# RenYurui/Global-Flow-Local-Attention

Hardware: AMD Instinct MI355X
Metric: images/sec (fwd+bwd) PoseGenerator 256x176 attn_layer=2,3 -- feature-warping hot path (higher is better)
Workload: dtype f32 (FC products: 2-term f16 splits exact to 2^-24 on f16 MFMA, f32 accumulate)

## Files before the change

### global_flow_local_attention_amd/csrc/patch_mfma.hip

```cpp
#include "gfla_common.h"
#include "patch_mfma.h"
#include "rs_taps.h"

namespace gfla {

typedef float pm_f32x16 __attribute__((ext_vector_type(16)));

struct PatchEntry {
  int q;
  float v;
};

constexpr int kPmStatSlots = 32;
constexpr int kPmTile = 32;
constexpr int kPmSub = 8;
constexpr int kPmChannels = 128;
constexpr int kPmMaxNB = 6;
constexpr int kPmGPitch = 33;

struct PmLayout {
  int64_t ntiles, table_bytes, rows_bytes, total;
};
static PmLayout pm_layout(int64_t B, int64_t HW, int entries) {
  PmLayout L;
  L.ntiles = ceil_div(HW, kPmTile);
  L.table_bytes = ((B * L.ntiles * kPmTile * entries * (int64_t)sizeof(PatchEntry)) + 255) & ~(int64_t)255;
  L.rows_bytes = ((B * L.ntiles * (int64_t)sizeof(int2)) + 255) & ~(int64_t)255;
  L.total = L.table_bytes + L.rows_bytes + 256;
  return L;
}

__device__ __forceinline__ unsigned pm_stat_total(const unsigned *stat) {
  unsigned tot = 0;
#pragma unroll
  for (int i = 0; i < kPmStatSlots; ++i) tot += stat[i];
  return tot;
}

__device__ __forceinline__ int pm_safe_int(float v) {
  return (int)fminf(fmaxf(v, -1048576.f), 1048576.f);
}

__device__ __forceinline__ void pm_store_tile_rows(int lo, int hi, int2 *slot, unsigned *stat) {
  __shared__ int s_lo[4], s_hi[4];
#pragma unroll
  for (int m = 32; m >= 1; m >>= 1) {
    lo = min(lo, __shfl_xor(lo, m));
    hi = max(hi, __shfl_xor(hi, m));
  }
  if ((threadIdx.x & 63) == 0) {
    s_lo[threadIdx.x >> 6] = lo;
    s_hi[threadIdx.x >> 6] = hi;
  }
  __syncthreads();
  if (threadIdx.x == 0) {
    const int l = min(min(s_lo[0], s_lo[1]), min(s_lo[2], s_lo[3])), h = max(max(s_hi[0], s_hi[1]), max(s_hi[2], s_hi[3]));
    *slot = make_int2(l, h);
    if (h >= l) atomicAdd(stat + (blockIdx.x + blockIdx.y * gridDim.x) % kPmStatSlots, (unsigned)(h - l + 1));
  }
}

struct Fold {
  int r_lo, r_hi, s_lo, s_hi, ty, tx;
  bool canonical;
};
__device__ __forceinline__ Fold pm_fold(int r, int s, int y0, int x0, int P, int Hs, int Ws) {
  Fold f;
  const int yy = y0 + r, xx = x0 + s;
  f.r_lo = f.r_hi = r;
  f.s_lo = f.s_hi = s;
  f.canonical = true;
  if (yy <= 0) {
    f.r_lo = 0;
    f.canonical = f.canonical && (yy == 0 || r == P - 1);
  } else if (yy >= Hs - 1) {
    f.r_hi = P - 1;
    f.canonical = f.canonical && (yy == Hs - 1 || r == 0);
  }
  if (xx <= 0) {
    f.s_lo = 0;
    f.canonical = f.canonical && (xx == 0 || s == P - 1);
  } else if (xx >= Ws - 1) {
    f.s_hi = P - 1;
    f.canonical = f.canonical && (xx == Ws - 1 || s == 0);
  }
  f.ty = clampi(yy, 0, Hs - 1);
  f.tx = clampi(xx, 0, Ws - 1);
  return f;
}

template <int K>
struct AggTaps {
  float fx0, fy0;
  int xf, yf, x0, y0;
  bool dense;
  __device__ __forceinline__ float dx(int t) const { return (fx0 + (float)(t - K / 2)) + (float)xf; }
  __device__ __forceinline__ float dy(int t) const { return (fy0 + (float)(t - K / 2)) + (float)yf; }
  __device__ __forceinline__ float ax(int t) const { const float d = dx(t); return d - floorf(d); }
  __device__ __forceinline__ float ay(int t) const { const float d = dy(t); return d - floorf(d); }
  __device__ __forceinline__ void init(float fx, float fy, int x, int y) {
    fx0 = fx, fy0 = fy, xf = x, yf = y;
    dense = true;
    x0 = y0 = 0;
#pragma unroll
    for (int t = 0; t < K; ++t) {
      const int ix = (int)floorf(dx(t)), iy = (int)floorf(dy(t));
      if (t == 0) x0 = ix, y0 = iy;
      dense = dense && (ix == x0 + t) && (iy == y0 + t);
    }
  }
};

template <int K>
__global__ __launch_bounds__(256) void agg_patch_table_kernel(const float *__restrict__ flow,
                                                             const float *__restrict__ attn,
                                                             PatchEntry *__restrict__ table,
                                                             int2 *__restrict__ tile_rows,
                                                             unsigned *__restrict__ stat, int H, int W, int Hs, int Ws,
                                                             int ntiles) {
  constexpr int P = K + 1, E = P * P, KK = K * K;
  static_assert(E % 2 == 0, "entries are written two at a time");
  typedef int i32x4 __attribute__((ext_vector_type(4)));
  const int64_t b = blockIdx.y;
  const int HW = H * W;
  const int tile = blockIdx.x * 8 + (threadIdx.x >> 5), pl = threadIdx.x & 31;
  if (tile >= ntiles) return;
  const int p = tile * kPmTile + pl;
  const float inv_kk = 1.f / (float)KK;
  int lo = 0x7fffffff, hi = -1;
  i32x4 *out = reinterpret_cast<i32x4 *>(table + ((b * ntiles + tile) * kPmTile + pl) * (int64_t)E);
  bool dense = false;
  AggTaps<K> tp;
  if (p < HW) {
    const int yf = p / W, xf = p - yf * W;
    tp.init(flow[(b * 2 + 0) * HW + p], flow[(b * 2 + 1) * HW + p], xf, yf);
    dense = tp.dense;
  }
  if (dense) {
    const int y0 = pm_safe_int((float)tp.y0), x0 = pm_safe_int((float)tp.x0);
    lo = clampi(y0, 0, Hs - 1);
    hi = clampi(y0 + K, 0, Hs - 1);
    float a[KK];
    const float *at = attn + b * (int64_t)KK * HW + p;
#pragma unroll
    for (int t = 0; t < KK; ++t) a[t] = at[(int64_t)t * HW] * inv_kk;
    float ax[K], ay[K];
#pragma unroll
    for (int t = 0; t < K; ++t) {
      ax[t] = tp.ax(t);
      ay[t] = tp.ay(t);
    }
    float v[P][P];
#pragma unroll
    for (int r = 0; r < P; ++r) {
#pragma unroll
      for (int q = 0; q < P; ++q) v[r][q] = 0.f;
#pragma unroll
      for (int j = 0; j < K; ++j) {
        float wrow = 0.f;
        if (r < K) wrow += a[r * K + j] * (1.f - ay[r]);
        if (r > 0) wrow += a[(r - 1) * K + j] * ay[r - 1];
        v[r][j] += wrow * (1.f - ax[j]);
        v[r][j + 1] += wrow * ax[j];
      }
    }
    int clo[P], chi[P], rlo[P], rhi[P], tx[P], ty[P];
    bool ccan[P], rcan[P];
#pragma unroll
    for (int i = 0; i < P; ++i) {
      const int xx = x0 + i, yy = y0 + i;
      clo[i] = chi[i] = rlo[i] = rhi[i] = i;
      ccan[i] = rcan[i] = true;
      if (xx <= 0) {
        clo[i] = 0;
        ccan[i] = xx == 0 || i == P - 1;
      } else if (xx >= Ws - 1) {
        chi[i] = P - 1;
        ccan[i] = xx == Ws - 1 || i == 0;
      }
      if (yy <= 0) {
        rlo[i] = 0;
        rcan[i] = yy == 0 || i == P - 1;
      } else if (yy >= Hs - 1) {
        rhi[i] = P - 1;
        rcan[i] = yy == Hs - 1 || i == 0;
      }
      tx[i] = clampi(xx, 0, Ws - 1);
      ty[i] = clampi(yy, 0, Hs - 1);
    }
    float cf[P][P];
#pragma unroll
    for (int r = 0; r < P; ++r)
#pragma unroll
      for (int q = 0; q < P; ++q) {
        float acc = 0.f;
#pragma unroll
        for (int q2 = 0; q2 < P; ++q2) acc += (q2 >= clo[q] && q2 <= chi[q]) ? v[r][q2] : 0.f;
        cf[r][q] = acc;
      }
#pragma unroll
    for (int r = 0; r < P; ++r)
#pragma unroll
      for (int q = 0; q < P; q += 2) {
        float acc0 = 0.f, acc1 = 0.f;
#pragma unroll
        for (int r2 = 0; r2 < P; ++r2) {
          const bool in = r2 >= rlo[r] && r2 <= rhi[r];
          acc0 += in ? cf[r2][q] : 0.f;
          acc1 += in ? cf[r2][q + 1] : 0.f;
        }
        const bool c0 = rcan[r] && ccan[q], c1 = rcan[r] && ccan[q + 1];
        i32x4 e;
        e.x = c0 ? (ty[r] << 16) | tx[q] : -1;
        e.y = c0 ? __float_as_int(acc0) : 0;
        e.z = c1 ? (ty[r] << 16) | tx[q + 1] : -1;
        e.w = c1 ? __float_as_int(acc1) : 0;
        out[(r * P + q) >> 1] = e;
      }
  } else {
    const i32x4 none = {-1, 0, -1, 0};
#pragma unroll
    for (int e = 0; e < E / 2; ++e) out[e] = none;
  }
#pragma unroll
  for (int msk = 16; msk >= 1; msk >>= 1) {
    lo = min(lo, __shfl_xor(lo, msk));
    hi = max(hi, __shfl_xor(hi, msk));
  }
  if (pl == 0) {
    tile_rows[b * ntiles + tile] = make_int2(lo, hi);
    if (hi >= lo) atomicAdd(stat + (tile + (int)b * ntiles) % kPmStatSlots, (unsigned)(hi - lo + 1));
  }
}

template <int K>
__global__ __launch_bounds__(256) void agg_scatter_nondense_kernel(const float *__restrict__ flow,
                                                                  const float *__restrict__ attn,
                                                                  const float *__restrict__ gout,
                                                                  float *__restrict__ gsrc, int C, int H, int W,
                                                                  int Hs, int Ws, const unsigned *__restrict__ stat,
                                                                  unsigned limit) {
  constexpr int KK = K * K;
  const int HW = H * W;
  if (pm_stat_total(stat) > limit) return;
  const int p = blockIdx.x * 256 + threadIdx.x;
  const int64_t b = blockIdx.y;
  if (p >= HW) return;
  const int yf = p / W, xf = p - yf * W;
  AggTaps<K> tp;
  tp.init(flow[(b * 2 + 0) * HW + p], flow[(b * 2 + 1) * HW + p], xf, yf);
  if (tp.dense) return;
  const float *at = attn + b * (int64_t)KK * HW + p;
  const float inv_kk = 1.f / (float)KK;
  for (int c = 0; c < C; ++c) {
    const float go = gout[(b * C + c) * (int64_t)HW + p] * inv_kk;
    float *gp = gsrc + (b * C + c) * (int64_t)Hs * Ws;
#pragma unroll 1
    for (int i = 0; i < K; ++i) {
      const float dy = tp.dy(i), fdy = floorf(dy);
      const int yT = clampi(pm_safe_int(fdy), 0, Hs - 1) * Ws, yB = clampi(pm_safe_int(fdy + 1), 0, Hs - 1) * Ws;
      const float yB_P = dy - fdy, yT_P = 1.f - yB_P;
#pragma unroll 1
      for (int j = 0; j < K; ++j) {
        const float dx = tp.dx(j), fdx = floorf(dx);
        const int xL = clampi(pm_safe_int(fdx), 0, Ws - 1), xR = clampi(pm_safe_int(fdx + 1), 0, Ws - 1);
        const float xR_P = dx - fdx, xL_P = 1.f - xR_P;
        const float gv = at[(int64_t)(i * K + j) * HW] * go;
        atomic_add(gp + yT + xL, gv * xL_P * yT_P);
        atomic_add(gp + yT + xR, gv * xR_P * yT_P);
        atomic_add(gp + yB + xL, gv * xL_P * yB_P);
        atomic_add(gp + yB + xR, gv * xR_P * yB_P);
      }
    }
  }
}

template <int KH>
__global__ __launch_bounds__(256) void rs_patch_table_kernel(const float *__restrict__ in2,
                                                            PatchEntry *__restrict__ table,
                                                            int2 *__restrict__ tile_rows,
                                                            unsigned *__restrict__ stat, int H, int W, int Hi, int Wi,
                                                            int trunc) {
  constexpr int P = 2 * KH, E = P * P;
  const int tile = blockIdx.x, ntiles = gridDim.x;
  const int64_t b = blockIdx.y;
  const int HW = H * W;
  const int pl = threadIdx.x >> 3, sub = threadIdx.x & (kPmSub - 1);
  const int p = tile * kPmTile + pl;
  PatchEntry *out = table + ((b * ntiles + tile) * kPmTile + pl) * (int64_t)E;
  int lo = 0x7fffffff, hi = -1;
  if (p < HW) {
    const int y = p / W, x = p - y * W;
    const float *i2 = in2 + b * 3 * (int64_t)HW + p;
    Taps<float, KH> t;
    t.template init<2>(i2[0], i2[HW], i2[2 * (int64_t)HW], x, y, Hi, Wi, 1, trunc != 0);
    const int y0 = pm_safe_int((float)t.iy0) - (KH - 1), x0 = pm_safe_int((float)t.ix0) - (KH - 1);
    lo = clampi(y0, 0, Hi - 1);
    hi = clampi(y0 + P - 1, 0, Hi - 1);
    float wy[P], wx[P];
#pragma unroll
    for (int r = 0; r < P; ++r) {
      wy[r] = (float)safe_div<float>(t.row_w(r), t.sum);
      wx[r] = t.col_w(r);
    }
    for (int e = sub; e < E; e += kPmSub) {
      const int r = e / P, s = e - r * P;
      const Fold f = pm_fold(r, s, y0, x0, P, Hi, Wi);
      float v = 0.f;
      if (f.canonical) {
#pragma unroll
        for (int rr = 0; rr < P; ++rr)
#pragma unroll
          for (int ss = 0; ss < P; ++ss)
            if (rr >= f.r_lo && rr <= f.r_hi && ss >= f.s_lo && ss <= f.s_hi) v += wy[rr] * wx[ss];
      }
      out[e] = f.canonical ? PatchEntry{(f.ty << 16) | f.tx, v} : PatchEntry{-1, 0.f};
    }
  } else {
    for (int e = sub; e < E; e += kPmSub) out[e] = PatchEntry{-1, 0.f};
  }
  pm_store_tile_rows(lo, hi, tile_rows + b * ntiles + tile, stat);
}

constexpr int kPmMaxEntriesPerThread = 5;

typedef float pm_f32x4 __attribute__((ext_vector_type(4)));

__device__ __forceinline__ void pm_fetch(pm_f32x4 (&gv)[4], int (&peq)[kPmMaxEntriesPerThread],
                                         float (&pev)[kPmMaxEntriesPerThread], int tile, const float *g_row, bool g_ok,
                                         bool g_vec, int gh, int HW, const PatchEntry *tab, int sub, int E) {
  const int pbase = tile * kPmTile + gh * 16;
#pragma unroll
  for (int q = 0; q < 4; ++q) {
    const int p = pbase + 4 * q;
    pm_f32x4 v = {0.f, 0.f, 0.f, 0.f};
    if (g_ok) {
      const float *src = g_row + (int64_t)tile * kPmTile + 4 * q;
      if (g_vec && p + 3 < HW) {
        v = *reinterpret_cast<const pm_f32x4 *>(src);
      } else {
        if (p < HW) v[0] = src[0];
        if (p + 1 < HW) v[1] = src[1];
        if (p + 2 < HW) v[2] = src[2];
        if (p + 3 < HW) v[3] = src[3];
      }
    }
    gv[q] = v;
  }
  const unsigned long long *tp = reinterpret_cast<const unsigned long long *>(tab + (int64_t)tile * kPmTile * E);
#pragma unroll
  for (int m = 0; m < kPmMaxEntriesPerThread; ++m) {
    const int e = sub + kPmSub * m;
    unsigned long long raw = 0xffffffffull;
    if (e < E) raw = tp[e];
    peq[m] = (int)(unsigned)(raw & 0xffffffffull);
    pev[m] = __uint_as_float((unsigned)(raw >> 32));
  }
}

template <int NB>
__global__ __launch_bounds__(256, 2) void patch_scatter_mfma_kernel(const float *__restrict__ G, float *__restrict__ dS,
                                                                   const PatchEntry *__restrict__ table,
                                                                   const int2 *__restrict__ tile_rows, int C, int HW,
                                                                   int Hs, int Ws, int R, int ntiles, int E,
                                                                   int accumulate, const unsigned *__restrict__ stat,
                                                                   unsigned limit) {
  constexpr int NQ = NB * 32;
  constexpr bool kSkip = NB >= 3;
  if (pm_stat_total(stat) > limit) return;
  extern __shared__ __attribute__((aligned(16))) unsigned char gfla_smem[];
  float *wt = reinterpret_cast<float *>(gfla_smem);
  float *gt = wt + kPmTile * NQ;
  unsigned short *list = reinterpret_cast<unsigned short *>(gt + kPmChannels * kPmGPitch);
  __shared__ int s_nlist;
  __shared__ unsigned s_mask[3];
  const int t = threadIdx.x, lane = t & 63, wave = t >> 6, l31 = lane & 31, kh = lane >> 5;
  const int band = blockIdx.x;
  const int64_t b = blockIdx.y;
  const int c0 = blockIdx.z * kPmChannels;
  const int by0 = band * R, by1 = min(Hs, by0 + R) - 1;
  const int nq = (by1 - by0 + 1) * Ws;

  if (wave == 0) {
    const int2 *tr = tile_rows + b * ntiles;
    int n = 0;
    for (int base = 0; base < ntiles; base += 64) {
      const int tile = base + lane;
      bool f = false;
      if (tile < ntiles) {
        const int2 rr = tr[tile];
        f = rr.x <= by1 && rr.y >= by0;
      }
      const unsigned long long m = __ballot(f);
      if (f) list[n + __popcll(m & ((1ull << lane) - 1ull))] = (unsigned short)tile;
      n += __popcll(m);
    }
    if (lane == 0) s_nlist = n;
  }
  __syncthreads();
  const int nlist = s_nlist;

  pm_f32x16 acc[NB];
#pragma unroll
  for (int j = 0; j < NB; ++j)
#pragma unroll
    for (int r = 0; r < 16; ++r) acc[j][r] = 0.f;

  const int gc = t >> 1, gh = t & 1;
  const bool g_ok = c0 + gc < C;
  const float *g_row = G + (b * C + (g_ok ? c0 + gc : 0)) * (int64_t)HW + gh * 16;
  const bool g_vec = (HW & 3) == 0 && (reinterpret_cast<uintptr_t>(G) & 15) == 0;
  const int pl = t >> 3, sub = t & (kPmSub - 1);
  const PatchEntry *tab = table + (b * ntiles * kPmTile + pl) * (int64_t)E;

  pm_f32x4 gv[4];
  int peq[kPmMaxEntriesPerThread];
  float pev[kPmMaxEntriesPerThread];
  if (nlist > 0) pm_fetch(gv, peq, pev, list[0], g_row, g_ok, g_vec, gh, HW, tab, sub, E);
  for (int li = 0; li < nlist; ++li) {
    __syncthreads();
#pragma unroll
    for (int i = 0; i < NB; ++i) reinterpret_cast<float4 *>(wt)[t + 256 * i] = make_float4(0.f, 0.f, 0.f, 0.f);
    if (kSkip && t < 3) s_mask[t] = 0u;
    {
      float *dst = gt + gc * kPmGPitch + gh * 16;
#pragma unroll
      for (int q = 0; q < 4; ++q) {
        dst[4 * q + 0] = gv[q][0];
        dst[4 * q + 1] = gv[q][1];
        dst[4 * q + 2] = gv[q][2];
        dst[4 * q + 3] = gv[q][3];
      }
    }
    __syncthreads();
    unsigned blocks = 0;
#pragma unroll
    for (int m = 0; m < kPmMaxEntriesPerThread; ++m) {
      const int q = peq[m];
      if (q >= 0) {
        const int ty = q >> 16, tx = q & 0xffff;
        if (ty >= by0 && ty <= by1) {
          const int col = (ty - by0) * Ws + tx;
          wt[pl * NQ + col] = pev[m];
          blocks |= 1u << (col >> 5);
        }
      }
    }
    if constexpr (kSkip) {
      blocks |= (unsigned)__shfl_xor((int)blocks, 1);
      blocks |= (unsigned)__shfl_xor((int)blocks, 2);
      blocks |= (unsigned)__shfl_xor((int)blocks, 4);
      blocks |= (unsigned)__shfl_xor((int)blocks, 8);
    }
    if (kSkip && (t & 15) == 0 && blocks) {
      const int base = (t >> 4) * NB, w = base >> 5, sh = base & 31;
      atomicOr(&s_mask[w], blocks << sh);
      if (sh + NB > 32) atomicOr(&s_mask[w + 1], blocks >> (32 - sh));
    }
    if (li + 1 < nlist)
      pm_fetch(gv, peq, pev, list[li + 1], g_row, g_ok, g_vec, gh, HW, tab, sub, E);
    __syncthreads();
    const unsigned mk0 = kSkip ? (unsigned)__builtin_amdgcn_readfirstlane((int)s_mask[0]) : 0xffffffffu;
    const unsigned mk1 = kSkip ? (unsigned)__builtin_amdgcn_readfirstlane((int)s_mask[1]) : 0xffffffffu;
    const unsigned mk2 = kSkip ? (unsigned)__builtin_amdgcn_readfirstlane((int)s_mask[2]) : 0xffffffffu;
    const float *ga = gt + (wave * 32 + l31) * kPmGPitch + kh;
    const float *wb = wt + kh * NQ + l31;
    float a = ga[0];
    float bq[NB];
#pragma unroll
    for (int j = 0; j < NB; ++j) bq[j] = wb[32 * j];
#pragma unroll 4
    for (int ks = 0; ks < kPmTile / 2; ++ks) {
      const float ac = a;
      float bc[NB];
#pragma unroll
      for (int j = 0; j < NB; ++j) bc[j] = bq[j];
      const int kn = ks + 1 < kPmTile / 2 ? ks + 1 : ks;
      a = ga[2 * kn];
#pragma unroll
      for (int j = 0; j < NB; ++j) bq[j] = wb[2 * kn * NQ + 32 * j];
      __builtin_amdgcn_sched_barrier(0);
#pragma unroll
      for (int j = 0; j < NB; ++j)
      {
        const int bit = ks * NB + j;
        const unsigned w = bit < 32 ? mk0 : (bit < 64 ? mk1 : mk2);
        if (!kSkip || ((w >> (bit & 31)) & 1u)) acc[j] = __builtin_amdgcn_mfma_f32_32x32x2f32(ac, bc[j], acc[j], 0, 0, 0);
      }
    }
  }
  const int64_t plane = (int64_t)Hs * Ws;
  const int cb = c0 + wave * 32 + 4 * kh;
  float *ob = dS + ((b * C + cb) * (int64_t)Hs + by0) * Ws + l31;
#pragma unroll
  for (int j = 0; j < NB; ++j) {
    const bool col_ok = 32 * j + l31 < nq;
    float oldv[16];
#pragma unroll
    for (int r = 0; r < 16; ++r) {
      const int dc = (r & 3) + 8 * (r >> 2);
      const bool ok = col_ok && cb + dc < C;
      oldv[r] = (accumulate && ok) ? ob[dc * plane + 32 * j] : 0.f;
    }
#pragma unroll
    for (int r = 0; r < 16; ++r) {
      const int dc = (r & 3) + 8 * (r >> 2);
      if (col_ok && cb + dc < C) ob[dc * plane + 32 * j] = oldv[r] + acc[j][r];
    }
  }
}

struct PmGeo {
  int R, NB, bands;
};
static PmGeo pm_geometry(int64_t B, int64_t C, int Hs, int Ws, int W, int patch) {
  (void)B, (void)C, (void)W, (void)patch;
  int R = tuning(13) > 0 ? tuning(13) : 96 / Ws;
  if (tuning(13) <= 0 && R < 2) R = (kPmMaxNB * 32) / Ws;
  if (R < 1) R = 1;
  if (R > Hs) R = Hs;
  while (R > 1 && R * Ws > kPmMaxNB * 32) --R;
  if (R * Ws > kPmMaxNB * 32) return PmGeo{0, 0, 0};
  return PmGeo{R, (int)ceil_div((int64_t)R * Ws, 32), (int)ceil_div(Hs, R)};
}

static bool pm_auto(bool aggregate, int64_t Ws) {
  if (tuning(14) == 2) return true;
  return aggregate ? true : Ws <= 24;
}

static int64_t pm_lds_bytes(int NB, int64_t ntiles) {
  return (int64_t)(kPmTile * NB * 32 + kPmChannels * kPmGPitch) * (int64_t)sizeof(float) + ((ntiles + 7) & ~(int64_t)7) * 2;
}

static bool pm_supported(int64_t B, int64_t C, int64_t H, int64_t W, int64_t Hs, int64_t Ws) {
  if (!(B > 0 && B <= 65535 && C > 0 && Hs >= 2 && Ws >= 2 && Ws <= kPmMaxNB * 32 && Hs < 32768 && Ws < 32768 &&
        H * W <= (int64_t)kPmTile * 65535 && ceil_div(C, kPmChannels) <= 65535 && tuning(14) != 1))
    return false;
  const PmGeo g = pm_geometry(B, C, (int)Hs, (int)Ws, (int)W, 0);
  return g.R > 0 && pm_lds_bytes(g.NB, ceil_div(H * W, kPmTile)) <= 64 * 1024;
}

static int pm_scatter(const float *G, float *dS, const PatchEntry *table, const int2 *tile_rows, int64_t B, int64_t C,
                      int64_t H, int64_t W, int64_t Hs, int64_t Ws, int entries, int patch, int accumulate,
                      const unsigned *stat, unsigned limit, hipStream_t stream) {
  const PmGeo g = pm_geometry(B, C, (int)Hs, (int)Ws, (int)W, patch);
  if (g.R == 0) return GFLA_ERR_UNSUPPORTED;
  const int ntiles = (int)ceil_div(H * W, kPmTile);
  const dim3 grid((unsigned)g.bands, (unsigned)B, (unsigned)ceil_div(C, kPmChannels));
  const unsigned lds = (unsigned)pm_lds_bytes(g.NB, ntiles);
  if (lds > 64 * 1024) return GFLA_ERR_UNSUPPORTED;
#define GFLA_PM(NB_)                                                                                              \
  case NB_:                                                                                                       \
    patch_scatter_mfma_kernel<NB_><<<grid, 256, lds, stream>>>(G, dS, table, tile_rows, (int)C, (int)(H * W), (int)Hs, \
                                                               (int)Ws, g.R, ntiles, entries, accumulate, stat, limit); \
    break
  switch (g.NB) {
    GFLA_PM(1);
    GFLA_PM(2);
    GFLA_PM(3);
    GFLA_PM(4);
    GFLA_PM(5);
    GFLA_PM(6);
    default: return GFLA_ERR_UNSUPPORTED;
  }
#undef GFLA_PM
  return launch_status();
}

static unsigned pm_limit(int64_t B, int64_t ntiles, int W, int patch, bool adaptive) {
  if (!adaptive || tuning(15) >= 100000) return 0xffffffffu;
  const double still = (double)kPmTile / W + 1.0 + patch;
  const double per_tile = tuning(15) > 0 ? (double)tuning(15) : 2.6 * still;
  const double total = per_tile * (double)B * (double)ntiles;
  return total >= 4.0e9 ? 0xffffffffu : (unsigned)total;
}

int agg_source_bwd_mfma(const float *flow, const float *attn, const float *gout, float *gsrc, void *workspace,
                        int64_t B, int64_t C, int64_t Hs, int64_t Ws, int64_t H, int64_t W, int k, int accumulate,
                        int adaptive, const unsigned **skip_stat, unsigned *skip_limit, hipStream_t stream) {
  if ((k != 3 && k != 5) || !pm_supported(B, C, H, W, Hs, Ws) || !workspace || !pm_auto(true, Ws)) return GFLA_ERR_UNSUPPORTED;
  const int entries = (k + 1) * (k + 1);
  const PmLayout L = pm_layout(B, H * W, entries);
  unsigned char *ws = static_cast<unsigned char *>(workspace);
  PatchEntry *table = reinterpret_cast<PatchEntry *>(ws);
  int2 *rows = reinterpret_cast<int2 *>(ws + L.table_bytes);
  unsigned *stat = reinterpret_cast<unsigned *>(ws + L.table_bytes + L.rows_bytes);
  const unsigned limit = pm_limit(B, L.ntiles, (int)W, k + 1, adaptive != 0);
  if (hipMemsetAsync(stat, 0, kPmStatSlots * 4, stream) != hipSuccess) return GFLA_ERR_LAUNCH;
  const dim3 tg((unsigned)ceil_div(L.ntiles, 8), (unsigned)B);
  if (k == 3)
    agg_patch_table_kernel<3><<<tg, 256, 0, stream>>>(flow, attn, table, rows, stat, (int)H, (int)W, (int)Hs, (int)Ws, (int)L.ntiles);
  else
    agg_patch_table_kernel<5><<<tg, 256, 0, stream>>>(flow, attn, table, rows, stat, (int)H, (int)W, (int)Hs, (int)Ws, (int)L.ntiles);
  int st = launch_status();
  if (st != GFLA_OK) return st;
  st = pm_scatter(gout, gsrc, table, rows, B, C, H, W, Hs, Ws, entries, k + 1, accumulate, stat, limit, stream);
  if (st != GFLA_OK) return st;
  const dim3 ng((unsigned)ceil_div(H * W, 256), (unsigned)B);
  if (k == 3)
    agg_scatter_nondense_kernel<3><<<ng, 256, 0, stream>>>(flow, attn, gout, gsrc, (int)C, (int)H, (int)W, (int)Hs, (int)Ws, stat, limit);
  else
    agg_scatter_nondense_kernel<5><<<ng, 256, 0, stream>>>(flow, attn, gout, gsrc, (int)C, (int)H, (int)W, (int)Hs, (int)Ws, stat, limit);
  if (skip_stat) *skip_stat = stat;
  if (skip_limit) *skip_limit = limit;
  return launch_status();
}

int rs_input1_bwd_mfma(const float *in2, const float *gout, float *gin1, void *workspace, int64_t B, int64_t C,
                       int64_t Hi, int64_t Wi, int64_t H, int64_t W, int k, int trunc, int accumulate, int adaptive,
                       const unsigned **skip_stat, unsigned *skip_limit, hipStream_t stream) {
  if ((k != 2 && k != 4) || !pm_supported(B, C, H, W, Hi, Wi) || !workspace || !pm_auto(false, Wi)) return GFLA_ERR_UNSUPPORTED;
  const int entries = k * k;
  const PmLayout L = pm_layout(B, H * W, entries);
  unsigned char *ws = static_cast<unsigned char *>(workspace);
  PatchEntry *table = reinterpret_cast<PatchEntry *>(ws);
  int2 *rows = reinterpret_cast<int2 *>(ws + L.table_bytes);
  unsigned *stat = reinterpret_cast<unsigned *>(ws + L.table_bytes + L.rows_bytes);
  const unsigned limit = pm_limit(B, L.ntiles, (int)W, k, adaptive != 0);
  if (hipMemsetAsync(stat, 0, kPmStatSlots * 4, stream) != hipSuccess) return GFLA_ERR_LAUNCH;
  const dim3 tg((unsigned)L.ntiles, (unsigned)B);
  if (k == 2)
    rs_patch_table_kernel<1><<<tg, 256, 0, stream>>>(in2, table, rows, stat, (int)H, (int)W, (int)Hi, (int)Wi, trunc);
  else
    rs_patch_table_kernel<2><<<tg, 256, 0, stream>>>(in2, table, rows, stat, (int)H, (int)W, (int)Hi, (int)Wi, trunc);
  const int st = launch_status();
  if (st != GFLA_OK) return st;
  if (skip_stat) *skip_stat = stat;
  if (skip_limit) *skip_limit = limit;
  return pm_scatter(gout, gin1, table, rows, B, C, H, W, Hi, Wi, entries, k, accumulate, stat, limit, stream);
}

int64_t pm_table_bytes(int64_t B, int64_t H, int64_t W, int entries) {
  if (B <= 0 || H <= 0 || W <= 0 || entries <= 0) return 0;
  return (pm_layout(B, H * W, entries).total + 255) & ~(int64_t)255;
}
int64_t pm_workspace_bytes(int64_t B, int64_t H, int64_t W, int entries) {
  if (B <= 0 || H <= 0 || W <= 0 || entries <= 0) return 0;
  return pm_table_bytes(B, H, W, entries) + B * H * W * kRsTapRecBytes;
}

}

extern "C" {
int64_t gfla_scatter_workspace_bytes(int64_t B, int64_t H, int64_t W, int patch_entries) {
  return gfla::pm_workspace_bytes(B, H, W, patch_entries);
}
}
```

Baseline: 9608.

## Double-buffer patch weight tiles and feed MFMA A operands from registers

Restructures the MFMA patch-scatter kernel so the G operand no longer goes through LDS. Each lane loads its own channel row and uses permlane32_swap to form the A operands in registers. The weight tile is double-buffered in LDS with an XOR-swizzled column-major layout, which allows vectorized B loads. Only previously written entries are cleared instead of zeroing the whole tile, and per-k block masks replace atomicOr bitmasks. This drops one barrier per tile and overlaps building the next tile with the current MFMA work, at the cost of more registers and double the weight LDS.

```diff
diff --git a/global_flow_local_attention_amd/csrc/patch_mfma.hip b/global_flow_local_attention_amd/csrc/patch_mfma.hip
--- a/global_flow_local_attention_amd/csrc/patch_mfma.hip
+++ b/global_flow_local_attention_amd/csrc/patch_mfma.hip
@@ -16,7 +16,6 @@
 constexpr int kPmSub = 8;
 constexpr int kPmChannels = 128;
 constexpr int kPmMaxNB = 6;
-constexpr int kPmGPitch = 33;
 
 struct PmLayout {
   int64_t ntiles, table_bytes, rows_bytes, total;
@@ -326,9 +325,13 @@
 
 typedef float pm_f32x4 __attribute__((ext_vector_type(4)));
 
-__device__ __forceinline__ void pm_fetch(pm_f32x4 (&gv)[4], int (&peq)[kPmMaxEntriesPerThread],
-                                         float (&pev)[kPmMaxEntriesPerThread], int tile, const float *g_row, bool g_ok,
-                                         bool g_vec, int gh, int HW, const PatchEntry *tab, int sub, int E) {
+__device__ __forceinline__ int pm_w_addr(int col, int pl) {
+  const int slot = ((pl & 1) << 4) | (pl >> 1);
+  return col * kPmTile + ((((slot >> 2) ^ (col >> 1)) & 7) << 2) + (slot & 3);
+}
+
+__device__ __forceinline__ void pm_fetch_g(pm_f32x4 (&gv)[4], int tile, const float *g_row, bool g_ok, bool g_vec, int gh,
+                                           int HW) {
   const int pbase = tile * kPmTile + gh * 16;
 #pragma unroll
   for (int q = 0; q < 4; ++q) {
@@ -347,6 +350,10 @@
     }
     gv[q] = v;
   }
+}
+
+__device__ __forceinline__ void pm_fetch_tab(int (&peq)[kPmMaxEntriesPerThread], float (&pev)[kPmMaxEntriesPerThread],
+                                             int tile, const PatchEntry *tab, int sub, int E) {
   const unsigned long long *tp = reinterpret_cast<const unsigned long long *>(tab + (int64_t)tile * kPmTile * E);
 #pragma unroll
   for (int m = 0; m < kPmMaxEntriesPerThread; ++m) {
@@ -355,6 +362,16 @@
     if (e < E) raw = tp[e];
     peq[m] = (int)(unsigned)(raw & 0xffffffffull);
     pev[m] = __uint_as_float((unsigned)(raw >> 32));
+  }
+}
+
+__device__ __forceinline__ void pm_a_operands(float (&a)[16], const pm_f32x4 (&gv)[4]) {
+#pragma unroll
+  for (int i = 0; i < 8; ++i) {
+    const float ev = gv[i >> 1][(2 * i) & 3], od = gv[i >> 1][(2 * i + 1) & 3];
+    const auto r = __builtin_amdgcn_permlane32_swap(__float_as_uint(ev), __float_as_uint(od), false, false);
+    a[i] = __uint_as_float(r[0]);
+    a[8 + i] = __uint_as_float(r[1]);
   }
 }
 
@@ -366,14 +383,14 @@
                                                                    int accumulate, const unsigned *__restrict__ stat,
                                                                    unsigned limit) {
   constexpr int NQ = NB * 32;
+  constexpr int kWFloats = kPmTile * NQ;
   constexpr bool kSkip = NB >= 3;
   if (pm_stat_total(stat) > limit) return;
   extern __shared__ __attribute__((aligned(16))) unsigned char gfla_smem[];
   float *wt = reinterpret_cast<float *>(gfla_smem);
-  float *gt = wt + kPmTile * NQ;
-  unsigned short *list = reinterpret_cast<unsigned short *>(gt + kPmChannels * kPmGPitch);
+  unsigned short *list = reinterpret_cast<unsigned short *>(wt + 2 * kWFloats);
   __shared__ int s_nlist;
-  __shared__ unsigned s_mask[3];
+  __shared__ unsigned s_kmask[2][kPmTile / 2];
   const int t = threadIdx.x, lane = t & 63, wave = t >> 6, l31 = lane & 31, kh = lane >> 5;
   const int band = blockIdx.x;
   const int64_t b = blockIdx.y;
@@ -397,6 +414,8 @@
     }
     if (lane == 0) s_nlist = n;
   }
+#pragma unroll
+  for (int i = 0; i < 2 * NB; ++i) reinterpret_cast<float4 *>(wt)[t + 256 * i] = make_float4(0.f, 0.f, 0.f, 0.f);
   __syncthreads();
   const int nlist = s_nlist;
 
@@ -406,88 +425,92 @@
 #pragma unroll
     for (int r = 0; r < 16; ++r) acc[j][r] = 0.f;
 
-  const int gc = t >> 1, gh = t & 1;
+  const int gc = wave * 32 + l31;
   const bool g_ok = c0 + gc < C;
-  const float *g_row = G + (b * C + (g_ok ? c0 + gc : 0)) * (int64_t)HW + gh * 16;
+  const float *g_row = G + (b * C + (g_ok ? c0 + gc : 0)) * (int64_t)HW + kh * 16;
   const bool g_vec = (HW & 3) == 0 && (reinterpret_cast<uintptr_t>(G) & 15) == 0;
   const int pl = t >> 3, sub = t & (kPmSub - 1);
   const PatchEntry *tab = table + (b * ntiles * kPmTile + pl) * (int64_t)E;
 
   pm_f32x4 gv[4];
+  float a[16];
   int peq[kPmMaxEntriesPerThread];
   float pev[kPmMaxEntriesPerThread];
-  if (nlist > 0) pm_fetch(gv, peq, pev, list[0], g_row, g_ok, g_vec, gh, HW, tab, sub, E);
-  for (int li = 0; li < nlist; ++li) {
-    __syncthreads();
-#pragma unroll
-    for (int i = 0; i < NB; ++i) reinterpret_cast<float4 *>(wt)[t + 256 * i] = make_float4(0.f, 0.f, 0.f, 0.f);
-    if (kSkip && t < 3) s_mask[t] = 0u;
-    {
-      float *dst = gt + gc * kPmGPitch + gh * 16;
-#pragma unroll
-      for (int q = 0; q < 4; ++q) {
-        dst[4 * q + 0] = gv[q][0];
-        dst[4 * q + 1] = gv[q][1];
-        dst[4 * q + 2] = gv[q][2];
-        dst[4 * q + 3] = gv[q][3];
-      }
-    }
-    __syncthreads();
+  int wa0[kPmMaxEntriesPerThread], wa1[kPmMaxEntriesPerThread];
+#pragma unroll
+  for (int m = 0; m < kPmMaxEntriesPerThread; ++m) wa0[m] = wa1[m] = -1;
+
+  auto build = [&](float *w, unsigned *km, int (&wa)[kPmMaxEntriesPerThread]) {
+#pragma unroll
+    for (int m = 0; m < kPmMaxEntriesPerThread; ++m)
+      if (wa[m] >= 0) w[wa[m]] = 0.f;
     unsigned blocks = 0;
 #pragma unroll
     for (int m = 0; m < kPmMaxEntriesPerThread; ++m) {
       const int q = peq[m];
+      int ad = -1;
       if (q >= 0) {
         const int ty = q >> 16, tx = q & 0xffff;
         if (ty >= by0 && ty <= by1) {
           const int col = (ty - by0) * Ws + tx;
-          wt[pl * NQ + col] = pev[m];
+          ad = pm_w_addr(col, pl);
+          w[ad] = pev[m];
           blocks |= 1u << (col >> 5);
         }
       }
+      wa[m] = ad;
     }
     if constexpr (kSkip) {
       blocks |= (unsigned)__shfl_xor((int)blocks, 1);
       blocks |= (unsigned)__shfl_xor((int)blocks, 2);
       blocks |= (unsigned)__shfl_xor((int)blocks, 4);
       blocks |= (unsigned)__shfl_xor((int)blocks, 8);
-    }
-    if (kSkip && (t & 15) == 0 && blocks) {
-      const int base = (t >> 4) * NB, w = base >> 5, sh = base & 31;
-      atomicOr(&s_mask[w], blocks << sh);
-      if (sh + NB > 32) atomicOr(&s_mask[w + 1], blocks >> (32 - sh));
-    }
-    if (li + 1 < nlist)
-      pm_fetch(gv, peq, pev, list[li + 1], g_row, g_ok, g_vec, gh, HW, tab, sub, E);
+      if ((t & 15) == 0) km[t >> 4] = blocks;
+    }
+  };
+  auto multiply = [&](const float *w, const unsigned *km) {
+    const int mine = kSkip ? (int)km[lane & 15] : 0;
+    unsigned mk[kPmTile / 2];
+#pragma unroll
+    for (int ks = 0; ks < kPmTile / 2; ++ks) mk[ks] = kSkip ? (unsigned)__builtin_amdgcn_readlane(mine, ks) : 0xffffffffu;
+    const float *wb = w + l31 * kPmTile;
+    const int sw = (l31 >> 1) & 7;
+#pragma unroll
+    for (int j = 0; j < NB; ++j) {
+      pm_f32x4 bq[4];
+#pragma unroll
+      for (int m = 0; m < 4; ++m)
+        bq[m] = *reinterpret_cast<const pm_f32x4 *>(wb + j * 32 * kPmTile + (((kh * 4 + m) ^ sw) << 2));
+#pragma unroll
+      for (int ks = 0; ks < kPmTile / 2; ++ks)
+        if (!kSkip || ((mk[ks] >> j) & 1u))
+          acc[j] = __builtin_amdgcn_mfma_f32_32x32x2f32(a[ks], bq[ks >> 2][ks & 3], acc[j], 0, 0, 0);
+    }
+  };
+  auto step = [&](int li, float *wc, unsigned *kc, float *wn, unsigned *kn, int (&wan)[kPmMaxEntriesPerThread]) {
+    const bool more = li + 1 < nlist, more2 = li + 2 < nlist;
+    if (more) build(wn, kn, wan);
+    if (more2) pm_fetch_tab(peq, pev, list[li + 2], tab, sub, E);
+    multiply(wc, kc);
+    if (more) pm_a_operands(a, gv);
+    if (more2) pm_fetch_g(gv, list[li + 2], g_row, g_ok, g_vec, kh, HW);
     __syncthreads();
-    const unsigned mk0 = kSkip ? (unsigned)__builtin_amdgcn_readfirstlane((int)s_mask[0]) : 0xffffffffu;
-    const unsigned mk1 = kSkip ? (unsigned)__builtin_amdgcn_readfirstlane((int)s_mask[1]) : 0xffffffffu;
-    const unsigned mk2 = kSkip ? (unsigned)__builtin_amdgcn_readfirstlane((int)s_mask[2]) : 0xffffffffu;
-    const float *ga = gt + (wave * 32 + l31) * kPmGPitch + kh;
-    const float *wb = wt + kh * NQ + l31;
-    float a = ga[0];
-    float bq[NB];
-#pragma unroll
-    for (int j = 0; j < NB; ++j) bq[j] = wb[32 * j];
-#pragma unroll 4
-    for (int ks = 0; ks < kPmTile / 2; ++ks) {
-      const float ac = a;
-      float bc[NB];
-#pragma unroll
-      for (int j = 0; j < NB; ++j) bc[j] = bq[j];
-      const int kn = ks + 1 < kPmTile / 2 ? ks + 1 : ks;
-      a = ga[2 * kn];
-#pragma unroll
-      for (int j = 0; j < NB; ++j) bq[j] = wb[2 * kn * NQ + 32 * j];
-      __builtin_amdgcn_sched_barrier(0);
-#pragma unroll
-      for (int j = 0; j < NB; ++j)
-      {
-        const int bit = ks * NB + j;
-        const unsigned w = bit < 32 ? mk0 : (bit < 64 ? mk1 : mk2);
-        if (!kSkip || ((w >> (bit & 31)) & 1u)) acc[j] = __builtin_amdgcn_mfma_f32_32x32x2f32(ac, bc[j], acc[j], 0, 0, 0);
-      }
-    }
+  };
+
+  if (nlist > 0) {
+    pm_fetch_g(gv, list[0], g_row, g_ok, g_vec, kh, HW);
+    pm_fetch_tab(peq, pev, list[0], tab, sub, E);
+    build(wt, s_kmask[0], wa0);
+    pm_a_operands(a, gv);
+    if (nlist > 1) {
+      pm_fetch_g(gv, list[1], g_row, g_ok, g_vec, kh, HW);
+      pm_fetch_tab(peq, pev, list[1], tab, sub, E);
+    }
+    __syncthreads();
+  }
+  for (int li = 0; li < nlist; li += 2) {
+    step(li, wt, s_kmask[0], wt + kWFloats, s_kmask[1], wa1);
+    if (li + 1 < nlist) step(li + 1, wt + kWFloats, s_kmask[1], wt, s_kmask[0], wa0);
   }
   const int64_t plane = (int64_t)Hs * Ws;
   const int cb = c0 + wave * 32 + 4 * kh;
@@ -530,7 +553,7 @@
 }
 
 static int64_t pm_lds_bytes(int NB, int64_t ntiles) {
-  return (int64_t)(kPmTile * NB * 32 + kPmChannels * kPmGPitch) * (int64_t)sizeof(float) + ((ntiles + 7) & ~(int64_t)7) * 2;
+  return (int64_t)(2 * kPmTile * NB * 32) * (int64_t)sizeof(float) + ((ntiles + 7) & ~(int64_t)7) * 2;
 }
 
 static bool pm_supported(int64_t B, int64_t C, int64_t H, int64_t W, int64_t Hs, int64_t Ws) {
```

Result: no change. 9630, median of 2 (+0.2%).
